# jackyko1991/vnet-tensorflow

Hardware: AMD Instinct MI355X
Metric: training patches/sec (128^3x1ch fp32) (higher is better)
Workload: dtype f32

## Files before the change

### vnet_tensorflow_amd/_lib.py

```python
import ctypes
import os
import subprocess

_HERE = os.path.dirname(os.path.abspath(__file__))
LIB_PATH = os.environ.get("VNET_HIP_LIB") or os.path.join(_HERE, "libvnet_hip.so")
CSRC = os.path.join(_HERE, "csrc")

_vp, _i, _i64, _f, _sz, _u64, _d = (ctypes.c_void_p, ctypes.c_int, ctypes.c_int64, ctypes.c_float,
                                    ctypes.c_size_t, ctypes.c_uint64, ctypes.c_double)

SIGNATURES = {
    "vnet_version": (ctypes.c_char_p, []),
    "vnet_set_option": (_d, [ctypes.c_char_p, _d]),
    "vnet_get_option": (_d, [ctypes.c_char_p]),
    "vnet_packed_weight_floats": (_sz, [_i, _i, _i, _i]),
    "vnet_pack_weights": (_i, [_i, _vp, _vp, _i, _i, _i, _vp]),
    "vnet_packed_dims": (_i, [_i, _i, _i, _i, ctypes.POINTER(ctypes.c_int), ctypes.POINTER(ctypes.c_int)]),
    "vnet_pack_weights_batched": (_i, [_vp, _i, _vp]),
    "vnet_conv_x3_ok": (_i, [_i] * 8),
    "vnet_conv_x3_stats_rows": (_i, [_i] * 6),
    "vnet_conv_x3_ws_bytes": (_sz, [_i] * 6),
    "vnet_conv_fwd_x3": (_i, [_vp, _i, _vp, _i, _vp, _vp, _vp, _i, _vp, _i, _i, _i, _i, _i, _vp, _vp, _vp, _vp, _sz, _vp]),
    "vnet_wgrad_x3_ok": (_i, [_i] * 7),
    "vnet_wgrad_x3_ws_bytes": (_sz, [_i] * 6),
# ... 85 lines not shown
    "vnet_bn_act_bwd_apply_b16": (_i, [_vp, _vp, _vp, _i, _i64, _i, _vp, _vp, _vp, _vp, _i, _vp, _vp, _vp, _d, _vp, _vp, _vp]),
    "vnet_bn_small_ok": (_i, [_i64, _i]),
    "vnet_bn_small_fwd_b16": (_i, [_vp, _vp, _i64, _i, _f, _f, _vp, _vp, _i, _vp, _vp, _vp, _vp, _vp, _vp, _vp]),
    "vnet_bn_small_bwd_b16": (_i, [_vp, _vp, _vp, _i64, _i, _vp, _vp, _vp, _vp, _i, _vp, _vp, _vp, _vp, _vp, _vp]),
    "vnet_head_fwd_b16": (_i, [_vp, _vp, _vp, _vp, _i64, _i, _i, _vp]),
    "vnet_head_bwd_b16": (_i, [_vp, _vp, _vp, _vp, _vp, _vp, _i64, _i, _i, _vp, _sz, _vp]),
    "vnet_dropout_fwd_b16": (_i, [_vp, _vp, _vp, _i64, _f, _u64, _vp, _vp]),
    "vnet_dropout_bwd_b16": (_i, [_vp, _vp, _vp, _i64, _f, _vp]),
}

SIGNATURES_UNET = {
    "vnet_maxpool2_fwd": (_i, [_vp, _vp, _i, _i, _i, _i, _i, _vp]),
    "vnet_maxpool2_bwd": (_i, [_vp, _vp, _vp, _vp, _i, _i, _i, _i, _i, _i, _vp]),
}


class WgradJob(ctypes.Structure):
    _fields_ = [("x0", ctypes.c_void_p), ("x1", ctypes.c_void_p), ("dy", ctypes.c_void_p), ("dw", ctypes.c_void_p),
                ("ws", ctypes.c_void_p), ("ws_bytes", ctypes.c_size_t),
                ("C0", ctypes.c_int), ("C1", ctypes.c_int), ("Cout", ctypes.c_int), ("Cin_dw", ctypes.c_int),
                ("B", ctypes.c_int), ("D", ctypes.c_int), ("H", ctypes.c_int), ("W", ctypes.c_int), ("ks", ctypes.c_int)]


ERRORS = {-1: "VNET_E_BADARG", -2: "VNET_E_UNSUPPORTED", -3: "VNET_E_WORKSPACE"}


def set_option(name, value):
    prev = lib().vnet_set_option(name.encode(), float(value))
    if prev != prev:
        raise VnetHipError("unknown library option %r" % (name,))
# ... 21 lines not shown
def lib():
    global _lib
    if _lib is None:
        if not os.path.exists(LIB_PATH):
            raise VnetHipError("libvnet_hip.so not found at %s -- run `python -c 'import __graft_entry__ as g; g.build()'` "
                               "(hipcc, gfx950).  The HIP library is the only compute path." % LIB_PATH)
        import torch
        L = ctypes.CDLL(LIB_PATH)
        for name, (res, args) in SIGNATURES.items():
            fn = getattr(L, name)
            fn.restype, fn.argtypes = res, args
            if name == "vnet_conv_b16_stats_rows":
                setattr(L, name, _memo(fn, (b"BF16_DEEP", b"BF16_DEEP_TARGET"), L))
            elif name.endswith("_ws_bytes") or name.endswith("_stats_rows") or name == "vnet_conv_stats_from_reduce" or name == "vnet_packed_weight_floats":
                setattr(L, name, _memo(fn))
        for name, (res, args) in SIGNATURES_UNET.items():
            fn = getattr(L, name)
            fn.restype, fn.argtypes = res, args
        _lib = L
    return _lib


_MEMOS = []


def _memo(fn, opts=None, L=None):
    cache = {}
    _MEMOS.append(cache)

    def cached(*args):
        key = args if opts is None else args + tuple(L.vnet_get_option(o) for o in opts)
        r = cache.get(key)
        if r is None:
# ... 9 lines not shown
```

### vnet_tensorflow_amd/csrc/elementwise.hip

```cpp
#include "common.h"

namespace {

#ifndef VNET_BN_RED_U
#define VNET_BN_RED_U 2
#endif
constexpr int EW_BLOCK = 256;
#ifndef VNET_EW_MAXBLK
#define VNET_EW_MAXBLK 1024
#endif
constexpr int EW_MAXBLK = VNET_EW_MAXBLK;
constexpr int MAXC = 1024;

inline int ew_blocks(size_t work_items) {
    size_t b = (work_items + EW_BLOCK - 1) / EW_BLOCK;
    if (b < 1) b = 1;
    if (b > EW_MAXBLK) b = EW_MAXBLK;
    return (int)b;
}
inline bool is_pow2(int v) { return v > 0 && (v & (v - 1)) == 0; }

__device__ __forceinline__ float act_fwd(float z, int act, float al) {
    if (act == VNET_ACT_RELU) return fmaxf(z, 0.f);
    if (act == VNET_ACT_PRELU) return fmaxf(z, 0.f) + al * fminf(z, 0.f);
// ... 485 lines not shown
        const float4 v = x[idx];
        acc[0].x += v.x; acc[0].y += v.y; acc[0].z += v.z; acc[0].w += v.w;
    }
    block_reduce_vec<1>(acc, CQ, CQ * 4, partial + (size_t)blockIdx.x * CQ * 4);
}
__global__ void __launch_bounds__(EW_BLOCK) colsum_generic_kernel(const float* __restrict__ x, size_t n, int C, float* __restrict__ partial) {
    __shared__ float sh[MAXC];
    for (int c = threadIdx.x; c < C; c += EW_BLOCK) sh[c] = 0.f;
    __syncthreads();
    const size_t stride = (size_t)gridDim.x * EW_BLOCK;
    for (size_t idx = (size_t)blockIdx.x * EW_BLOCK + threadIdx.x; idx < n; idx += stride) atomicAdd(&sh[idx % C], x[idx]);
    __syncthreads();
    for (int c = threadIdx.x; c < C; c += EW_BLOCK) partial[(size_t)blockIdx.x * C + c] = sh[c];
}

template <int K>
__global__ void __launch_bounds__(EW_BLOCK) head_fwd_kernel(const float* __restrict__ x, const float* __restrict__ w,
                                                            const float* __restrict__ bias, float* __restrict__ y, size_t M, int C) {
    __shared__ float ws[MAXC * 8 / 8];
    for (int t = threadIdx.x; t < C * K; t += EW_BLOCK) ws[t] = w[t];
    __syncthreads();
    const size_t stride = (size_t)gridDim.x * EW_BLOCK;
    for (size_t row = (size_t)blockIdx.x * EW_BLOCK + threadIdx.x; row < M; row += stride) {
        float o[K];
#pragma unroll
        for (int k = 0; k < K; ++k) o[k] = bias ? bias[k] : 0.f;
        const float* xr = x + row * C;
        if ((C & 3) == 0) {
            for (int c = 0; c < C; c += 4) {
                const float4 v = *reinterpret_cast<const float4*>(xr + c);
#pragma unroll
                for (int k = 0; k < K; ++k)
                    o[k] += v.x * ws[c * K + k] + v.y * ws[(c + 1) * K + k] + v.z * ws[(c + 2) * K + k] + v.w * ws[(c + 3) * K + k];
            }
        } else {
            for (int c = 0; c < C; ++c) {
                const float v = xr[c];
#pragma unroll
                for (int k = 0; k < K; ++k) o[k] += v * ws[c * K + k];
            }
        }
#pragma unroll
        for (int k = 0; k < K; ++k) y[row * K + k] = o[k];
    }
}

template <int K>
__global__ void __launch_bounds__(EW_BLOCK) head_bwd_kernel(const float* __restrict__ x, const float* __restrict__ w,
// ... 55 lines not shown
    for (size_t row = (size_t)blockIdx.x * EW_BLOCK + threadIdx.x; row < M; row += stride) {
        float g[K];
#pragma unroll
        for (int k = 0; k < K; ++k) { g[k] = dy[row * K + k]; atomicAdd(&acc[C * K + k], g[k]); }
        for (int c = 0; c < C; ++c) {
            const float v = x[row * C + c];
            float o = 0.f;
#pragma unroll
            for (int k = 0; k < K; ++k) { o += g[k] * ws[c * K + k]; atomicAdd(&acc[c * K + k], v * g[k]); }
            if (dx) dx[row * C + c] = o;
        }
    }
    __syncthreads();
    float* prow = partial + (size_t)blockIdx.x * (C * K + K);
    for (int t = threadIdx.x; t < C * K + K; t += EW_BLOCK) prow[t] = acc[t];
}

struct LossP {
    const float* logits; const int32_t* labels; const float* weights;
    float* softmax_out; long long* pred_out; float* partial;
    size_t V; int B; int K; int kind; int nblk;
};

template <int K>
__global__ void __launch_bounds__(EW_BLOCK) softmax_dice_fwd_kernel(LossP p) {
    const int b = blockIdx.y;
    const bool jac = (p.kind & 15) == VNET_LOSS_JACCARD;
    const bool wx = (p.kind & VNET_LOSS_WEIGHTED) && p.weights;
    float aI[K], aL[K], aR[K], aX = 0.f;
#pragma unroll
// ... 893 lines not shown
    const float sc = 1.f / (1.f - rate);
    for (size_t i = (size_t)blockIdx.x * blockDim.x + threadIdx.x; i < n8; i += (size_t)gridDim.x * blockDim.x) {
        float v[8];
        unpack8(dy[i], v);
        const uint2 m = reinterpret_cast<const uint2*>(mask)[i];
#pragma unroll
        for (int k = 0; k < 8; ++k) v[k] = (((k < 4 ? m.x : m.y) >> (8 * (k & 3))) & 0xffu) ? v[k] * sc : 0.f;
        dx[i] = pack8(v);
    }
}
}

template <typename F>
static int with_k(int K, F&& f) { return with_int<1, 2, 3, 4, 5, 6, 7, 8>(K, f); }
template <typename F>
static int with_bcast_r(bool bcast, bool hasr, F&& f) {
    return bcast ? f(std::true_type{}, std::false_type{}) : with_bool(hasr, [&](auto R) { return f(std::false_type{}, R); });
}

extern "C" {

size_t vnet_bn_ws_bytes(int C) { return (size_t)EW_MAXBLK * 3 * (C > 8 ? C : 8) * sizeof(float); }
size_t vnet_colsum_ws_bytes(int C) { return (size_t)EW_MAXBLK * (C > 8 ? C : 8) * sizeof(float); }
size_t vnet_head_ws_bytes(int C, int K) { return (size_t)EW_MAXBLK * (C * K + K) * sizeof(float); }
size_t vnet_loss_ws_bytes(int B, int K) { return (size_t)B * EW_MAXBLK * (3 * K + 1) * sizeof(float) + (size_t)B * (3 * K + 1) * sizeof(double) + 16; }

static int bn_partial_moments(const float* x, const float* r, int bcast, int64_t M, int C, float* partial, hipStream_t st, int* nblk_out) {
    const int Cs = bcast ? 1 : C;
    const int mode = red_mode(Cs);
    int nblk, e;
// ... 215 lines not shown
    float* partial = (float*)ws;
    int nblk, e;
    if ((C & 3) == 0 && is_pow2(C / 4) && C / 4 <= EW_BLOCK) {
        nblk = ew_blocks((size_t)M * (C / 4) / 4 + 1);
        e = with_k(K, [&](auto KK) {
            return launch<head_bwd_kernel<KK>>(dim3(nblk), dim3(EW_BLOCK), 0, st, x, w, dy, dx, (size_t)M, C, partial);
        });
    } else {
        nblk = ew_blocks((size_t)M / 4 + 1);
        e = with_k(K, [&](auto KK) {
            return launch<head_bwd_generic_kernel<KK>>(dim3(nblk), dim3(EW_BLOCK), 0, st, x, w, dy, dx, (size_t)M, C, partial);
        });
    }
    if (e) return e;
    return launch<head_finalize_kernel>(dim3(C * K + K), dim3(256), 0, st, partial, nblk, C * K, K, dw, db);
}

int vnet_softmax_dice_fwd(const float* logits, const int32_t* labels, int B, int64_t V, int K,
                          int loss_kind, const float* weights, float alpha, float smooth,
                          float* softmax_out, int64_t* pred_out, float* loss_out, float* dice_out,
                          float* coef, void* ws, size_t ws_bytes, void* stream) {
    if (!logits || !labels || !loss_out || !coef || B <= 0 || V <= 0 || K <= 0) return VNET_E_BADARG;
    if (B * K > 64 || B > 8) return VNET_E_UNSUPPORTED;
    if ((loss_kind & 15) > VNET_LOSS_XENT) return VNET_E_UNSUPPORTED;
    if ((loss_kind & VNET_LOSS_WEIGHTED) && !weights) return VNET_E_BADARG;
    if (!ws || ws_bytes < vnet_loss_ws_bytes(B, K)) return VNET_E_WORKSPACE;
    hipStream_t st = (hipStream_t)stream;
    LossP p{}; p.logits = logits; p.labels = labels; p.weights = weights; p.softmax_out = softmax_out;
    p.pred_out = (long long*)pred_out; p.partial = (float*)ws; p.V = (size_t)V; p.B = B; p.K = K; p.kind = loss_kind;
    const int nblk = ew_blocks((size_t)V / 4 + 1);
// ... 331 lines not shown
```

### vnet_tensorflow_amd/layers2.py

```python
import numpy as np

from . import ops
from ._scope import get_variable, variable_scope, current


def xavier_initializer_convolution(shape, dist='uniform', lambda_initializer=True):
    s = len(shape) - 2
    num_activations = np.prod(shape[:s]) * np.sum(shape[s:])
    if dist == 'uniform':
        lim = np.sqrt(6. / num_activations)
        return np.random.uniform(-lim, lim, shape).astype(np.float32)
    if dist == 'normal':
        stddev = np.sqrt(3. / num_activations)
        return np.random.normal(0, stddev, shape).astype(np.float32)
    raise ValueError('Distribution must be either "uniform" or "normal".')


def constant_initializer(value, shape, lambda_initializer=True):
    return np.full(shape, value).astype(np.float32)


def get_num_channels(x):
    return int(x.shape[-1])

# ... 101 lines not shown
    return ops.activation(x, "relu")


def leaky_relu(x):
    return ops.activation(x, "lrelu")


def convolution_tiled(tiled, filter, bn_stats=False, bn_residual=None):
    filter = list(filter)
    w = get_variable(name='weights', initializer=lambda: xavier_initializer_convolution(shape=filter))
    b = get_variable(name='biases', initializer=lambda: constant_initializer(0, shape=filter[-1]))
    img, gamma, beta, mean, invstd = tiled
    return ops.input_conv(img, gamma, beta, mean, invstd, w, b, bn_stats=bn_stats, bn_residual=bn_residual)


def batch_normalization(x, activation=None, residual=None, tile=False, channels=None, dead=False,
                        momentum=0.99, epsilon=0.001, want_stats=False):
    C = int(channels if channels is not None else x.shape[-1])
    gamma, beta, mm, mv = _bn_variables(C)
    if dead:
        ops.bn_update_only(x, C, mm, mv)
        return None
    alpha = None
    if activation == "prelu":
        alpha = get_variable('alpha', initializer=lambda: np.full((C,), 0.1, dtype=np.float32))
    if want_stats:
        y, mean, invstd = ops.bn_act(x, gamma, beta, activation, alpha, residual, tile, mm, mv, want_stats=True)
        return y, (x, gamma, beta, mean, invstd)
    return ops.bn_act(x, gamma, beta, activation, alpha, residual, tile, mm, mv)


def _bn_variables(C):
    store = current()
    with variable_scope(store.unique_layer_name("batch_normalization")):
        gamma = get_variable('gamma', initializer=lambda: np.ones((C,), np.float32))
        beta = get_variable('beta', initializer=lambda: np.zeros((C,), np.float32))
        mm = get_variable('moving_mean', initializer=lambda: np.zeros((C,), np.float32), trainable=False)
        mv = get_variable('moving_variance', initializer=lambda: np.ones((C,), np.float32), trainable=False)
    return gamma, beta, mm, mv


def batch_normalization_chain(x, kind, activation=None):
    C = int(x.shape[-1])
    layers = [_bn_variables(C) for _ in range(3 if kind == 0 else 2)]
    alpha = None
    if activation == "prelu":
        alpha = get_variable('alpha', initializer=lambda: np.full((C,), 0.1, dtype=np.float32))
    (g1, b1, mm1, mv1), (g2, b2, mm2, mv2) = layers[0], layers[1]
    g3 = b3 = mm3 = mv3 = None
    if kind == 0:
        g3, b3, mm3, mv3 = layers[2]
    return ops.bn_chain(x, kind, activation, alpha, g1, b1, g2, b2, g3, b3, (mm1, mv1, mm2, mv2, mm3, mv3))
```

### vnet_tensorflow_amd/networks.py

```python
import torch

from . import layers2 as L
from ._scope import VariableStore


class VNet(object):
    def __init__(self,
                 num_classes,
                 dropout_rate=0.01,
                 num_channels=16,
                 num_levels=4,
                 num_convolutions=(1, 2, 3, 3),
                 bottom_convolutions=3,
                 is_training=True,
                 activation_fn="relu",
                 device=None):
        self.num_classes = num_classes
        self.dropout_rate = dropout_rate
        self.num_channels = num_channels
        assert num_levels == len(num_convolutions)
        self.num_levels = num_levels
        self.num_convolutions = num_convolutions
        self.bottom_convolutions = bottom_convolutions
        self.is_training = is_training
        self.train_phase = True
        if activation_fn not in ("relu", "prelu", "lrelu"):
            raise ValueError("activation_fn must be relu, prelu or lrelu")
        self.activation_fn = activation_fn
        self.fuse_input_block = True
        self.fuse_bn_chains = True
        self.cut_backward = False
        self.backward_cuts = []
        self.fuse_bn_stats = True
        self.fuse_grad_accumulation = True
        self.fuse_zero_bias_grad = True
        self.variables = VariableStore(device)

    def parameters(self):
        return list(self.variables.params.values())

    def named_parameters(self):
        return list(self.variables.params.items())

    def state_dict(self):
        return self.variables.state_dict()

    def load_state_dict(self, sd):
        self.variables.load_state_dict(sd)

    def build(self, input_shape):
# ... 49 lines not shown
                        x = L.down_convolution(x, factor=2, kernel_size=[2, 2, 2], bn_stats=self.fuse_bn_stats)
                        x = L.batch_normalization(x, activation=act)

            if cutting:
                features = [ops.cut(f, self.backward_cuts) for f in features]
                x = ops.cut(x, self.backward_cuts)
            with store.variable_scope('vnet/bottom_level'):
                x = self.convolution_block(x, self.bottom_convolutions, dropout_rate, act)

            for l in reversed(range(self.num_levels)):
                with store.variable_scope('vnet/decoder/level_' + str(l + 1)):
                    f = features[l]
                    with store.variable_scope('up_convolution'):
                        x = L.up_convolution(x, tuple(f.shape), factor=2, kernel_size=[2, 2, 2])
                        x = L.batch_normalization(x, activation=act)
                    x = self.convolution_block_2(x, f, self.num_convolutions[l], dropout_rate, act)

            with store.variable_scope('vnet/output_layer'):
                logits = L.convolution(x, [1, 1, 1, self.num_channels, self.num_classes])
                logits = L.batch_normalization(logits)
        return logits

    def convolution_block(self, layer_input, num_convolutions, dropout_rate, activation_fn, is_training=True, tiled=None):
        from . import ops
        store = self.variables
        x = layer_input
        n_channels = L.get_num_channels(x)
        if tiled is None and self.fuse_grad_accumulation:
            x, layer_input = ops.fork(layer_input)
        for i in range(num_convolutions):
            with store.variable_scope('conv_' + str(i + 1)):
                res = layer_input if i == num_convolutions - 1 else None
                if i == 0 and tiled is not None:
                    x = L.convolution_tiled(tiled, [5, 5, 5, n_channels, n_channels], bn_stats=self.fuse_bn_stats, bn_residual=res)
                else:
                    x = L.convolution(x, [5, 5, 5, n_channels, n_channels], bn_stats=self.fuse_bn_stats, bn_residual=res)
                x = L.batch_normalization(x, activation=activation_fn, residual=res)
                x = ops.dropout(x, dropout_rate)
        return x

    def convolution_block_2(self, layer_input, fine_grained_features, num_convolutions, dropout_rate, activation_fn,
                            is_training=True):
        from . import ops
        store = self.variables
        n_channels = L.get_num_channels(layer_input)
        if num_convolutions == 1:
            with store.variable_scope('conv_' + str(1)):
                x = L.convolution_concat(layer_input, fine_grained_features, [5, 5, 5, n_channels * 2, n_channels], bn_stats=self.fuse_bn_stats)
                if self.fuse_bn_chains:
                    x = L.batch_normalization_chain(x, 0, activation_fn)
                else:
                    x = L.batch_normalization(x)
                    r = L.batch_normalization(x)
                    x = L.batch_normalization(x, activation=activation_fn, residual=r)
                x = ops.dropout(x, dropout_rate)
            return x

        with store.variable_scope('conv_' + str(1)):
            x = L.convolution_concat(layer_input, fine_grained_features, [5, 5, 5, n_channels * 2, n_channels], bn_stats=self.fuse_bn_stats)
            x = L.batch_normalization(x, activation=activation_fn)
            x = ops.dropout(x, dropout_rate)

        for i in range(1, num_convolutions):
            with store.variable_scope('conv_' + str(i + 1)):
                x = L.convolution(x, [5, 5, 5, n_channels, n_channels], bn_stats=self.fuse_bn_stats)
                last = (i == num_convolutions - 1)
                if last and self.fuse_bn_chains:
                    x = L.batch_normalization_chain(x, 1, activation_fn)
                else:
                    r = L.batch_normalization(x, dead=not last)
                    x = L.batch_normalization(x, activation=activation_fn, residual=r if last else None)
                x = ops.dropout(x, dropout_rate)
        return x


class UNet(object):

    def __init__(self,
                 num_output_channels,
                 dropout_rate=0.01,
                 num_channels=4,
                 num_levels=4,
                 num_convolutions=2,
                 bottom_convolutions=2,
                 is_training=True,
                 activation_fn="relu",
                 device=None):
# ... 102 lines not shown
```

### vnet_tensorflow_amd/ops.py

```python
import collections
import contextlib
import ctypes
import math
import os as _os
import weakref

import torch

from . import _lib
from ._lib import VnetHipError, check

BN_EPS = 1e-3
BN_MOMENTUM = 0.99

ACT = {None: 0, "none": 0, "relu": 1, "prelu": 2, "lrelu": 3}
PACK_FWD, PACK_BWD, PACK_UP, PACK_FWD_BF16, PACK_BWD_BF16, PACK_BOTH_BF16, PACK_BOTH = 0, 1, 2, 3, 4, 5, 6
PACK_FWD_X3, PACK_BWD_X3, PACK_BOTH_X3 = 7, 8, 9

class OpsContext(object):
    def __init__(self):
        self.compute = {"dtype": "fp32", "store16": False, "name": "fp32", "split3": False}
        self.pg = {"on": False, "streams": {}, "used": set(), "keep": []}
        self.pack_epoch = [0]
        self.pack_reg = {"entries": [], "descs": None, "device": None}
# ... 1022 lines not shown
        name = "vnet_bn_stats" + sfx
        check(getattr(L, name)(_ptr(x), _ptr(r), *tile, M, C, BN_EPS, BN_MOMENTUM, _ptr(mean), _ptr(invstd), _ptr(mm), _ptr(mv),
                               _ptr(ws), nb, _stream()), name)
        return mean, invstd, float(M)
    all_reduce, world = _SYNC_BN
    sums = torch.empty(2 * C, dtype=torch.float64, device=x.device)
    name = "vnet_bn_moments" + sfx
    check(getattr(L, name)(_ptr(x), _ptr(r), *tile, M, C, _ptr(sums), _ptr(ws), nb, _stream()), name)
    all_reduce(sums)
    check(L.vnet_bn_finalize(_ptr(sums), float(M) * world, C, BN_EPS, BN_MOMENTUM, _ptr(mean), _ptr(invstd),
                             _ptr(mm), _ptr(mv), _stream()), "vnet_bn_finalize")
    return mean, invstd, float(M) * world


def _bn_backward(rt, dy, x, r, bcast, M, C, mean, invstd, scale, shift, act, alpha, dscale, dshift, dalpha, ds, m_total,
                 all_reduce=None, coef=None):
    L = _lib.lib()
    nb = L.vnet_bn_ws_bytes(C)
    ws = workspace(nb, dy.device)
    if rt.stats == "small":
        check(L.vnet_bn_small_bwd_b16(_ptr(dy), _ptr(x), _ptr(r), M, C, _ptr(mean), _ptr(invstd), _ptr(scale), _ptr(shift), act,
                                      _ptr(alpha), _ptr(dscale), _ptr(dshift), _ptr(dalpha), _ptr(ds), _stream()), "vnet_bn_small_bwd_b16")
        return
    sfx = "_b16" if rt.apply16 else ""
    args = (_ptr(dy), _ptr(x), _ptr(r), int(bcast), M, C, _ptr(mean), _ptr(invstd), _ptr(scale), _ptr(shift), act, _ptr(alpha))
    name = "vnet_bn_act_bwd_reduce" + sfx
    check(getattr(L, name)(*args, _ptr(dscale), _ptr(dshift), _ptr(dalpha), _ptr(ws), nb, _stream()), name)
    sdz, sdzx = dshift, dscale
    if rt.allreduce and (ds is not None or coef is not None):
        sdz = torch.cat([dshift.reshape(-1), dscale.reshape(-1)])
        all_reduce(sdz)
        sdzx = sdz[C:]
    extra = coef(sdzx) if coef is not None else None
    if ds is not None:
        name = "vnet_bn_act_bwd_apply" + sfx
        check(getattr(L, name)(*args, _ptr(sdz), _ptr(sdzx), m_total, _ptr(extra), _ptr(ds), _stream()), name)


class _BnActFn(torch.autograd.Function):
    @staticmethod
    def forward(ctx, x, r, gamma, beta, alpha, act, bcast, mm, mv):
        L = _lib.lib()
# ... 311 lines not shown
            check(L.vnet_head_bwd_b16(_ptr(x), _ptr(w), _ptr(dy), _ptr(dx), _ptr(dw), _ptr(db), M, C, K, _ptr(ws), nb, _stream()),
                  "vnet_head_bwd_b16")
        else:
            check(L.vnet_head_bwd(_ptr(x), _ptr(w), _ptr(dy), _ptr(dx), _ptr(dw), _ptr(db), M, C, K, _ptr(ws), nb, _stream()),
                  "vnet_head_bwd")
        return dx, _grad_ret(dw, sw), _grad_ret(db, sb)


def head_conv(x, w, b):
    if _meta(x):
        return torch.empty(x.shape[:-1] + (w.shape[-1],), device="meta")
    _need_gpu(x, "head_conv", allow16=True)
    return _HeadFn.apply(x, w, b)


def parse_loss(name):
    valid = ("xent", "weighted_xent", "sorensen", "weighted_sorensen", "jaccard", "weighted_jaccard",
             "mixed_sorensen", "mixed_weighted_sorensen", "mixed_jaccard", "mixed_weighted_jaccard")
    if name not in valid:
        raise SystemExit("Invalid loss function")
    kind = LOSS_KIND["xent"] if name.endswith("xent") else (LOSS_KIND["sorensen"] if "sorensen" in name else LOSS_KIND["jaccard"])
    if "weighted" in name:
        kind |= LOSS_WEIGHTED
    if name.startswith("mixed_"):
        kind |= LOSS_MIXED
    return kind


_CONST_VEC = {}

# ... 240 lines not shown
```

Measured before the change: 65.46.

## Fuse final batch-norm+activation with the 1x1 head convolution in forward and backward

Adds fused HIP kernels that apply batch-norm plus activation and immediately compute the 1x1x1 head logits, so the normalized activation tensor is never written out for small channel counts (C=8 or 16). The backward path is fused too: one reduce kernel computes the BN gradient sums together with the head weight and bias gradients, and one apply kernel recomputes dy from dlogits and the head weights on the fly. The goal is to remove full-volume reads and writes of the intermediate activation and its gradient, plus several kernel launches. In exchange the kernels use cross-lane shuffles and larger per-thread register footprints, and the forward head dot product disables FMA contraction to match the unfused numerics.

```diff
diff --git a/include/vnet_hip_head.h b/include/vnet_hip_head.h
--- /dev/null
+++ b/include/vnet_hip_head.h
@@ -0,0 +1,28 @@
+#ifndef VNET_HIP_HEAD_H
+#define VNET_HIP_HEAD_H
+#include "vnet_hip.h"
+
+#ifdef __cplusplus
+extern "C" {
+#endif
+
+int vnet_bn_head_ok(int C, int K);
+int vnet_bn_head_stats_rows(int64_t M, int C);
+size_t vnet_bn_head_ws_bytes(int C, int K);
+
+int vnet_bn_act_head_fwd(const float* x, const float* r, int64_t M, int C,
+    const float* mean, const float* invstd, const float* gamma, const float* beta, int act, const float* alpha,
+    const float* w, const float* bias, int K, float* y, float* logits, float* stats, void* stream);
+
+int vnet_bn_act_bwd_reduce_head(const float* dlogits, const float* w, int K, const float* x, const float* r, int64_t M, int C,
+    const float* mean, const float* invstd, const float* gamma, const float* beta, int act, const float* alpha,
+    float* dgamma, float* dbeta, float* dalpha, float* dw, float* db, void* ws, size_t ws_bytes, void* stream);
+
+int vnet_bn_act_bwd_apply_head(const float* dlogits, const float* w, int K, const float* x, const float* r, int64_t M, int C,
+    const float* mean, const float* invstd, const float* gamma, const float* beta, int act, const float* alpha,
+    const float* sum_dz, const float* sum_dz_xhat, double M_total, const float* xhat_coef, float* ds, void* stream);
+
+#ifdef __cplusplus
+}
+#endif
+#endif
diff --git a/vnet_tensorflow_amd/_lib.py b/vnet_tensorflow_amd/_lib.py
--- a/vnet_tensorflow_amd/_lib.py
+++ b/vnet_tensorflow_amd/_lib.py
@@ -123,6 +123,16 @@
     "vnet_maxpool2_bwd": (_i, [_vp, _vp, _vp, _vp, _i, _i, _i, _i, _i, _i, _vp]),
 }
 
+SIGNATURES_HEAD = {
+    "vnet_bn_head_ok": (_i, [_i, _i]),
+    "vnet_bn_head_stats_rows": (_i, [_i64, _i]),
+    "vnet_bn_head_ws_bytes": (_sz, [_i, _i]),
+    "vnet_bn_act_head_fwd": (_i, [_vp, _vp, _i64, _i, _vp, _vp, _vp, _vp, _i, _vp, _vp, _vp, _i, _vp, _vp, _vp, _vp]),
+    "vnet_bn_act_bwd_reduce_head": (_i, [_vp, _vp, _i, _vp, _vp, _i64, _i, _vp, _vp, _vp, _vp, _i, _vp,
+                                         _vp, _vp, _vp, _vp, _vp, _vp, _sz, _vp]),
+    "vnet_bn_act_bwd_apply_head": (_i, [_vp, _vp, _i, _vp, _vp, _i64, _i, _vp, _vp, _vp, _vp, _i, _vp, _vp, _vp, _d, _vp, _vp, _vp]),
+}
+
 
 class WgradJob(ctypes.Structure):
     _fields_ = [("x0", ctypes.c_void_p), ("x1", ctypes.c_void_p), ("dy", ctypes.c_void_p), ("dw", ctypes.c_void_p),
@@ -174,9 +184,11 @@
                 setattr(L, name, _memo(fn, (b"BF16_DEEP", b"BF16_DEEP_TARGET"), L))
             elif name.endswith("_ws_bytes") or name.endswith("_stats_rows") or name == "vnet_conv_stats_from_reduce" or name == "vnet_packed_weight_floats":
                 setattr(L, name, _memo(fn))
-        for name, (res, args) in SIGNATURES_UNET.items():
+        for name, (res, args) in list(SIGNATURES_UNET.items()) + list(SIGNATURES_HEAD.items()):
             fn = getattr(L, name)
             fn.restype, fn.argtypes = res, args
+            if name in ("vnet_bn_head_ok", "vnet_bn_head_stats_rows", "vnet_bn_head_ws_bytes"):
+                setattr(L, name, _memo(fn))
         _lib = L
     return _lib
 
diff --git a/vnet_tensorflow_amd/csrc/elementwise.hip b/vnet_tensorflow_amd/csrc/elementwise.hip
--- a/vnet_tensorflow_amd/csrc/elementwise.hip
+++ b/vnet_tensorflow_amd/csrc/elementwise.hip
@@ -1,4 +1,5 @@
 #include "common.h"
+#include "../../include/vnet_hip_head.h"
 
 namespace {
 
@@ -523,6 +524,10 @@
     for (int c = threadIdx.x; c < C; c += EW_BLOCK) partial[(size_t)blockIdx.x * C + c] = sh[c];
 }
 
+__device__ __forceinline__ float head_quad_dot(const float4 v, float w0, float w1, float w2, float w3) {
+#pragma clang fp contract(off)
+    return v.x * w0 + v.y * w1 + v.z * w2 + v.w * w3;
+}
 template <int K>
 __global__ void __launch_bounds__(EW_BLOCK) head_fwd_kernel(const float* __restrict__ x, const float* __restrict__ w,
                                                             const float* __restrict__ bias, float* __restrict__ y, size_t M, int C) {
@@ -539,8 +544,7 @@
             for (int c = 0; c < C; c += 4) {
                 const float4 v = *reinterpret_cast<const float4*>(xr + c);
 #pragma unroll
-                for (int k = 0; k < K; ++k)
-                    o[k] += v.x * ws[c * K + k] + v.y * ws[(c + 1) * K + k] + v.z * ws[(c + 2) * K + k] + v.w * ws[(c + 3) * K + k];
+                for (int k = 0; k < K; ++k) o[k] += head_quad_dot(v, ws[c * K + k], ws[(c + 1) * K + k], ws[(c + 2) * K + k], ws[(c + 3) * K + k]);
             }
         } else {
             for (int c = 0; c < C; ++c) {
@@ -626,6 +630,218 @@
     __syncthreads();
     float* prow = partial + (size_t)blockIdx.x * (C * K + K);
     for (int t = threadIdx.x; t < C * K + K; t += EW_BLOCK) prow[t] = acc[t];
+}
+
+struct HeadP {
+    const float* w; const float* bias; const float* dl;
+    float* logits; float* stats; float* hpartial;
+};
+
+template <int K>
+__device__ __forceinline__ void head_load_row(const float* __restrict__ p, size_t row, float (&g)[K]) {
+    if constexpr (K == 2) { const float2 t = reinterpret_cast<const float2*>(p)[row]; g[0] = t.x; g[1] = t.y; }
+    else if constexpr (K == 4) { const float4 t = reinterpret_cast<const float4*>(p)[row]; g[0] = t.x; g[1] = t.y; g[2] = t.z; g[3] = t.w; }
+    else {
+#pragma unroll
+        for (int k = 0; k < K; ++k) g[k] = p[row * K + k];
+    }
+}
+template <int K>
+__device__ __forceinline__ void head_store_row(float* __restrict__ p, size_t row, const float (&g)[K]) {
+    if constexpr (K == 2) reinterpret_cast<float2*>(p)[row] = make_float2(g[0], g[1]);
+    else if constexpr (K == 4) reinterpret_cast<float4*>(p)[row] = make_float4(g[0], g[1], g[2], g[3]);
+    else {
+#pragma unroll
+        for (int k = 0; k < K; ++k) p[row * K + k] = g[k];
+    }
+}
+
+struct HeadQuad { float sc[4], sf[4], al[4], mu[4], is[4]; };
+template <int K>
+__device__ __forceinline__ void head_quad_load(const BnP& p, const HeadP& h, int c, const float* sc, const float* sf, const float* al,
+                                               HeadQuad& q, float (&wv)[4][K]) {
+#pragma unroll
+    for (int i = 0; i < 4; ++i) {
+        q.sc[i] = sc[c + i]; q.sf[i] = sf[c + i]; q.al[i] = al[c + i];
+        q.mu[i] = p.mean[c + i]; q.is[i] = p.invstd[c + i];
+#pragma unroll
+        for (int k = 0; k < K; ++k) wv[i][k] = h.w[(c + i) * K + k];
+    }
+}
+template <int K>
+__device__ __forceinline__ void head_quad_dy(const float (&g)[K], const float (&wv)[4][K], float (&dy)[4]) {
+    float4 o = make_float4(0, 0, 0, 0);
+#pragma unroll
+    for (int k = 0; k < K; ++k) {
+        o.x = fmaf(g[k], wv[0][k], o.x); o.y = fmaf(g[k], wv[1][k], o.y);
+        o.z = fmaf(g[k], wv[2][k], o.z); o.w = fmaf(g[k], wv[3][k], o.w);
+    }
+    dy[0] = o.x; dy[1] = o.y; dy[2] = o.z; dy[3] = o.w;
+}
+
+template <int K, int CQ>
+__global__ void __launch_bounds__(EW_BLOCK) bn_act_head_fwd_kernel(BnP p, HeadP h) {
+    __shared__ float sc[MAXC], sf[MAXC], al[MAXC];
+    bn_load_coef(p, sc, sf, al);
+    const size_t nq = p.M * CQ;
+    const size_t stride = (size_t)gridDim.x * EW_BLOCK;
+    const size_t start = (size_t)blockIdx.x * EW_BLOCK + threadIdx.x;
+    const int cq = (int)(start % CQ), c = cq * 4;
+    HeadQuad q; float wv[4][K], bias[K];
+    head_quad_load<K>(p, h, c, sc, sf, al, q, wv);
+#pragma unroll
+    for (int k = 0; k < K; ++k) bias[k] = h.bias ? h.bias[k] : 0.f;
+    float acc[2][8];
+#pragma unroll
+    for (int k = 0; k < 8; ++k) acc[0][k] = acc[1][k] = 0.f;
+    for (size_t idx = start; idx < nq; idx += stride) {
+        float4 v = reinterpret_cast<const float4*>(p.x)[idx];
+        if (p.r) { const float4 t = reinterpret_cast<const float4*>(p.r)[idx]; v.x += t.x; v.y += t.y; v.z += t.z; v.w += t.w; }
+        float4 o;
+        o.x = act_fwd(v.x * q.sc[0] + q.sf[0], p.act, q.al[0]);
+        o.y = act_fwd(v.y * q.sc[1] + q.sf[1], p.act, q.al[1]);
+        o.z = act_fwd(v.z * q.sc[2] + q.sf[2], p.act, q.al[2]);
+        o.w = act_fwd(v.w * q.sc[3] + q.sf[3], p.act, q.al[3]);
+        if (p.out) reinterpret_cast<float4*>(p.out)[idx] = o;
+        float part[K], lg[K];
+#pragma unroll
+        for (int k = 0; k < K; ++k) { part[k] = head_quad_dot(o, wv[0][k], wv[1][k], wv[2][k], wv[3][k]); lg[k] = bias[k]; }
+#pragma unroll
+        for (int j = 0; j < CQ; ++j)
+#pragma unroll
+            for (int k = 0; k < K; ++k) lg[k] += __shfl(part[k], j, CQ);
+        if (cq == 0) {
+            head_store_row<K>(h.logits, idx / CQ, lg);
+#pragma unroll
+            for (int k = 0; k < K; ++k) { acc[0][k] += lg[k]; acc[1][k] += lg[k] * lg[k]; }
+        }
+    }
+    if (h.stats) block_reduce_row<2, 8>(acc, K, h.stats + (size_t)blockIdx.x * 2 * K);
+}
+
+template <int K, int CQ>
+__global__ void __launch_bounds__(EW_BLOCK) bn_act_bwd_reduce_head_kernel(BnP p, HeadP h) {
+    __shared__ float sc[MAXC], sf[MAXC], al[MAXC];
+    __shared__ float shh[5 * K][EW_BLOCK];
+    bn_load_coef(p, sc, sf, al);
+    constexpr int C = 4 * CQ;
+    const size_t nq = p.M * CQ;
+    const size_t stride = (size_t)gridDim.x * EW_BLOCK;
+    const size_t start = (size_t)blockIdx.x * EW_BLOCK + threadIdx.x;
+    const int cq = (int)(start % CQ), c = cq * 4;
+    HeadQuad q; float wv[4][K];
+    head_quad_load<K>(p, h, c, sc, sf, al, q, wv);
+    float4 acc[3] = {make_float4(0, 0, 0, 0), make_float4(0, 0, 0, 0), make_float4(0, 0, 0, 0)};
+    float hs[5 * K];
+#pragma unroll
+    for (int s = 0; s < 5 * K; ++s) hs[s] = 0.f;
+    constexpr int U = VNET_BN_RED_U;
+    for (size_t idx = start; idx < nq; idx += U * stride) {
+        float4 v[U]; float g[U][K];
+#pragma unroll
+        for (int u = 0; u < U; ++u) {
+            const size_t j0 = idx + u * stride;
+            const bool ok = j0 < nq;
+            const size_t j = ok ? j0 : idx;
+            v[u] = reinterpret_cast<const float4*>(p.x)[j];
+            if (p.r) { const float4 t = reinterpret_cast<const float4*>(p.r)[j]; v[u].x += t.x; v[u].y += t.y; v[u].z += t.z; v[u].w += t.w; }
+            head_load_row<K>(h.dl, j / CQ, g[u]);
+            if (!ok) {
+#pragma unroll
+                for (int k = 0; k < K; ++k) g[u][k] = 0.f;
+            }
+        }
+#pragma unroll
+        for (int u = 0; u < U; ++u) {
+            const float vv[4] = {v[u].x, v[u].y, v[u].z, v[u].w};
+            float gg[4], a0[4], a1[4], a2[4];
+            head_quad_dy<K>(g[u], wv, gg);
+#pragma unroll
+            for (int i = 0; i < 4; ++i) {
+                const float z = vv[i] * q.sc[i] + q.sf[i];
+                const float dz = gg[i] * act_grad(z, p.act, q.al[i]);
+                const float xh = (vv[i] - q.mu[i]) * q.is[i];
+                a0[i] = dz; a1[i] = dz * xh; a2[i] = gg[i] * fminf(z, 0.f);
+                const float y = act_fwd(z, p.act, q.al[i]);
+#pragma unroll
+                for (int k = 0; k < K; ++k) hs[i * K + k] = fmaf(y, g[u][k], hs[i * K + k]);
+            }
+            acc[0].x += a0[0]; acc[0].y += a0[1]; acc[0].z += a0[2]; acc[0].w += a0[3];
+            acc[1].x += a1[0]; acc[1].y += a1[1]; acc[1].z += a1[2]; acc[1].w += a1[3];
+            acc[2].x += a2[0]; acc[2].y += a2[1]; acc[2].z += a2[2]; acc[2].w += a2[3];
+            if (cq == 0) {
+#pragma unroll
+                for (int k = 0; k < K; ++k) hs[4 * K + k] += g[u][k];
+            }
+        }
+    }
+    block_reduce_vec<3>(acc, CQ, C, p.partial + (size_t)blockIdx.x * 3 * C);
+#pragma unroll
+    for (int s = 0; s < 5 * K; ++s) shh[s][threadIdx.x] = hs[s];
+    __syncthreads();
+    if (threadIdx.x < 64) {
+        const int t = threadIdx.x;
+        float* prow = h.hpartial + (size_t)blockIdx.x * (C * K + K);
+#pragma unroll
+        for (int s = 0; s < 5 * K; ++s) {
+            float v = (shh[s][t] + shh[s][t + 128]) + (shh[s][t + 64] + shh[s][t + 192]);
+#pragma unroll
+            for (int o = 32; o >= CQ; o >>= 1) v += __shfl_down(v, o, 64);
+            if (s < 4 * K) { if (t < CQ) prow[(t * 4 + s / K) * K + s % K] = v; }
+            else if (t == 0) prow[C * K + s - 4 * K] = v;
+        }
+    }
+}
+
+template <int K, int CQ>
+__global__ void __launch_bounds__(EW_BLOCK) bn_act_bwd_apply_head_kernel(BnP p, HeadP h) {
+    __shared__ float sc[MAXC], sf[MAXC], al[MAXC];
+    bn_load_coef(p, sc, sf, al);
+    const size_t nq = p.M * CQ;
+    const size_t stride = (size_t)gridDim.x * EW_BLOCK;
+    const size_t start = (size_t)blockIdx.x * EW_BLOCK + threadIdx.x;
+    const int cq = (int)(start % CQ), c = cq * 4;
+    HeadQuad q; float wv[4][K], k1[4], k2[4], ex[4];
+    head_quad_load<K>(p, h, c, sc, sf, al, q, wv);
+#pragma unroll
+    for (int i = 0; i < 4; ++i) {
+        k1[i] = p.dbeta[c + i] * p.invM; k2[i] = p.dgamma[c + i] * p.invM;
+        ex[i] = p.extra ? p.extra[c + i] : 0.f;
+    }
+    for (size_t idx = start; idx < nq; idx += stride) {
+        float4 v = reinterpret_cast<const float4*>(p.x)[idx];
+        if (p.r) { const float4 t = reinterpret_cast<const float4*>(p.r)[idx]; v.x += t.x; v.y += t.y; v.z += t.z; v.w += t.w; }
+        float g[K], gg[4], o[4];
+        head_load_row<K>(h.dl, idx / CQ, g);
+        head_quad_dy<K>(g, wv, gg);
+        const float vv[4] = {v.x, v.y, v.z, v.w};
+#pragma unroll
+        for (int i = 0; i < 4; ++i) {
+            const float z = vv[i] * q.sc[i] + q.sf[i];
+            const float dz = gg[i] * act_grad(z, p.act, q.al[i]);
+            const float xh = (vv[i] - q.mu[i]) * q.is[i];
+            o[i] = q.sc[i] * (dz - k1[i] - xh * k2[i]) + xh * ex[i];
+        }
+        reinterpret_cast<float4*>(p.out)[idx] = make_float4(o[0], o[1], o[2], o[3]);
+    }
+}
+
+__global__ void __launch_bounds__(256) bn_head_finalize_kernel(const float* __restrict__ bnp, const float* __restrict__ hp, int nblk,
+                                                               int C, int CK, int K, float* o0, float* o1, float* o2, float* dw, float* db) {
+    if ((int)blockIdx.x < C) {
+        const int c = blockIdx.x;
+        double s[3];
+        block_colsum_multi<3>(bnp, nblk, (size_t)3 * C, c, C, s);
+        if (threadIdx.x == 0) {
+            if (o0) o0[c] = (float)s[0];
+            if (o1) o1[c] = (float)s[1];
+            if (o2) o2[c] = (float)s[2];
+        }
+        return;
+    }
+    const int c = blockIdx.x - C;
+    const double s = block_colsum_d(hp, nblk, (size_t)(CK + K), c);
+    if (threadIdx.x == 0) { if (c < CK) dw[c] = (float)s; else db[c - CK] = (float)s; }
 }
 
 struct LossP {
@@ -1549,6 +1765,10 @@
 template <typename F>
 static int with_k(int K, F&& f) { return with_int<1, 2, 3, 4, 5, 6, 7, 8>(K, f); }
 template <typename F>
+static int with_k_cq(int K, int C, F&& f) {
+    return with_k(K, [&](auto KK) { return with_int<2, 4>(C / 4, [&](auto CQ) { return f(KK, CQ); }); });
+}
+template <typename F>
 static int with_bcast_r(bool bcast, bool hasr, F&& f) {
     return bcast ? f(std::true_type{}, std::false_type{}) : with_bool(hasr, [&](auto R) { return f(std::false_type{}, R); });
 }
@@ -1794,6 +2014,65 @@
     }
     if (e) return e;
     return launch<head_finalize_kernel>(dim3(C * K + K), dim3(256), 0, st, partial, nblk, C * K, K, dw, db);
+}
+
+static inline bool bn_head_shape_ok(int C, int K) { return (C == 8 || C == 16) && K >= 1 && K <= 8; }
+static inline int bn_head_blocks(int64_t M, int C) { return ew_blocks((size_t)M * C / 4 / 4 + 1); }
+
+int vnet_bn_head_ok(int C, int K) { return bn_head_shape_ok(C, K) ? 1 : 0; }
+int vnet_bn_head_stats_rows(int64_t M, int C) { return (M > 0 && (C == 8 || C == 16)) ? bn_head_blocks(M, C) : 0; }
+size_t vnet_bn_head_ws_bytes(int C, int K) { return (size_t)EW_MAXBLK * (3 * C + C * K + K) * sizeof(float); }
+
+int vnet_bn_act_head_fwd(const float* x, const float* r, int64_t M, int C,
+                         const float* mean, const float* invstd, const float* gamma, const float* beta, int act, const float* alpha,
+                         const float* w, const float* bias, int K, float* y, float* logits, float* stats, void* stream) {
+    if (!x || !mean || !invstd || !gamma || !beta || !w || !logits || M <= 0) return VNET_E_BADARG;
+    if (act == VNET_ACT_PRELU && !alpha) return VNET_E_BADARG;
+    if (act < 0 || act > 3 || !bn_head_shape_ok(C, K)) return VNET_E_UNSUPPORTED;
+    BnP p{}; p.x = x; p.r = r; p.mean = mean; p.invstd = invstd; p.gamma = gamma; p.beta = beta; p.alpha = alpha;
+    p.out = y; p.M = (size_t)M; p.C = C; p.act = act;
+    HeadP h{}; h.w = w; h.bias = bias; h.logits = logits; h.stats = stats;
+    return with_k_cq(K, C, [&](auto KK, auto CQ) {
+        return launch<bn_act_head_fwd_kernel<KK, CQ>>(dim3(bn_head_blocks(M, C)), dim3(EW_BLOCK), 0, (hipStream_t)stream, p, h);
+    });
+}
+
+int vnet_bn_act_bwd_reduce_head(const float* dlogits, const float* w, int K, const float* x, const float* r, int64_t M, int C,
+                                const float* mean, const float* invstd, const float* gamma, const float* beta,
+                                int act, const float* alpha, float* dgamma, float* dbeta, float* dalpha, float* dw, float* db,
+                                void* ws, size_t ws_bytes, void* stream) {
+    if (!dlogits || !w || !x || !mean || !invstd || !gamma || !beta || !dgamma || !dbeta || !dw || !db || M <= 0) return VNET_E_BADARG;
+    if (act == VNET_ACT_PRELU && (!alpha || !dalpha)) return VNET_E_BADARG;
+    if (act < 0 || act > 3 || !bn_head_shape_ok(C, K)) return VNET_E_UNSUPPORTED;
+    if (!ws || ws_bytes < vnet_bn_head_ws_bytes(C, K)) return VNET_E_WORKSPACE;
+    hipStream_t st = (hipStream_t)stream;
+    BnP p{}; bn_bwd_fill(p, nullptr, x, r, 0, M, C, mean, invstd, gamma, beta, act, alpha);
+    p.partial = (float*)ws;
+    HeadP h{}; h.w = w; h.dl = dlogits; h.hpartial = p.partial + (size_t)EW_MAXBLK * 3 * C;
+    const int nblk = bn_head_blocks(M, C);
+    if (int e = with_k_cq(K, C, [&](auto KK, auto CQ) {
+            return launch<bn_act_bwd_reduce_head_kernel<KK, CQ>>(dim3(nblk), dim3(EW_BLOCK), 0, st, p, h); }))
+        return e;
+    return launch<bn_head_finalize_kernel>(dim3(C + C * K + K), dim3(256), 0, st, (const float*)p.partial, (const float*)h.hpartial, nblk,
+                                           C, C * K, K, dbeta, dgamma, act == VNET_ACT_PRELU ? dalpha : (float*)nullptr, dw, db);
+}
+
+int vnet_bn_act_bwd_apply_head(const float* dlogits, const float* w, int K, const float* x, const float* r, int64_t M, int C,
+                               const float* mean, const float* invstd, const float* gamma, const float* beta,
+                               int act, const float* alpha, const float* sum_dz, const float* sum_dz_xhat, double M_total,
+                               const float* xhat_coef, float* ds, void* stream) {
+    if (!dlogits || !w || !x || !mean || !invstd || !gamma || !beta || !sum_dz || !sum_dz_xhat || !ds || M <= 0 || M_total <= 0.0)
+        return VNET_E_BADARG;
+    if (act == VNET_ACT_PRELU && !alpha) return VNET_E_BADARG;
+    if (act < 0 || act > 3 || !bn_head_shape_ok(C, K)) return VNET_E_UNSUPPORTED;
+    BnP p{}; bn_bwd_fill(p, nullptr, x, r, 0, M, C, mean, invstd, gamma, beta, act, alpha);
+    p.invM = (float)(1.0 / M_total);
+    p.extra = xhat_coef;
+    p.out = ds; p.dgamma = sum_dz_xhat; p.dbeta = sum_dz;
+    HeadP h{}; h.w = w; h.dl = dlogits;
+    return with_k_cq(K, C, [&](auto KK, auto CQ) {
+        return launch<bn_act_bwd_apply_head_kernel<KK, CQ>>(dim3(bn_head_blocks(M, C)), dim3(EW_BLOCK), 0, (hipStream_t)stream, p, h);
+    });
 }
 
 int vnet_softmax_dice_fwd(const float* logits, const int32_t* labels, int B, int64_t V, int K,
diff --git a/vnet_tensorflow_amd/layers2.py b/vnet_tensorflow_amd/layers2.py
--- a/vnet_tensorflow_amd/layers2.py
+++ b/vnet_tensorflow_amd/layers2.py
@@ -139,8 +139,25 @@
     return ops.input_conv(img, gamma, beta, mean, invstd, w, b, bn_stats=bn_stats, bn_residual=bn_residual)
 
 
+class DeferredNorm(object):
+
+    def __init__(self, x, kind, activation, alpha, layers, residual=None):
+        self.x, self.kind, self.activation, self.alpha, self.layers, self.residual = x, kind, activation, alpha, layers, residual
+        self.shape = x.shape
+
+
+def convolution_after_norm(d, filter):
+    filter = list(filter)
+    assert filter[:3] == [1, 1, 1], filter
+    w = get_variable(name='weights', initializer=lambda: xavier_initializer_convolution(shape=filter))
+    b = get_variable(name='biases', initializer=lambda: constant_initializer(0, shape=filter[-1]))
+    g = [v for layer in d.layers for v in layer[:2]] + [None] * (6 - 2 * len(d.layers))
+    moving = [v for layer in d.layers for v in layer[2:]] + [None] * (6 - 2 * len(d.layers))
+    return ops.bn_head(d.x, w, b, d.kind, d.activation, d.alpha, *g, residual=d.residual, moving=tuple(moving))
+
+
 def batch_normalization(x, activation=None, residual=None, tile=False, channels=None, dead=False,
-                        momentum=0.99, epsilon=0.001, want_stats=False):
+                        momentum=0.99, epsilon=0.001, want_stats=False, defer=False):
     C = int(channels if channels is not None else x.shape[-1])
     gamma, beta, mm, mv = _bn_variables(C)
     if dead:
@@ -149,6 +166,9 @@
     alpha = None
     if activation == "prelu":
         alpha = get_variable('alpha', initializer=lambda: np.full((C,), 0.1, dtype=np.float32))
+    if defer:
+        assert not tile and not want_stats
+        return DeferredNorm(x, -1, activation, alpha, [(gamma, beta, mm, mv)], residual)
     if want_stats:
         y, mean, invstd = ops.bn_act(x, gamma, beta, activation, alpha, residual, tile, mm, mv, want_stats=True)
         return y, (x, gamma, beta, mean, invstd)
@@ -165,12 +185,14 @@
     return gamma, beta, mm, mv
 
 
-def batch_normalization_chain(x, kind, activation=None):
+def batch_normalization_chain(x, kind, activation=None, defer=False):
     C = int(x.shape[-1])
     layers = [_bn_variables(C) for _ in range(3 if kind == 0 else 2)]
     alpha = None
     if activation == "prelu":
         alpha = get_variable('alpha', initializer=lambda: np.full((C,), 0.1, dtype=np.float32))
+    if defer:
+        return DeferredNorm(x, kind, activation, alpha, layers)
     (g1, b1, mm1, mv1), (g2, b2, mm2, mv2) = layers[0], layers[1]
     g3 = b3 = mm3 = mv3 = None
     if kind == 0:
diff --git a/vnet_tensorflow_amd/networks.py b/vnet_tensorflow_amd/networks.py
--- a/vnet_tensorflow_amd/networks.py
+++ b/vnet_tensorflow_amd/networks.py
@@ -34,6 +34,7 @@
         self.fuse_bn_stats = True
         self.fuse_grad_accumulation = True
         self.fuse_zero_bias_grad = True
+        self.fuse_head = True
         self.variables = VariableStore(device)
 
     def parameters(self):
@@ -113,10 +114,14 @@
                     with store.variable_scope('up_convolution'):
                         x = L.up_convolution(x, tuple(f.shape), factor=2, kernel_size=[2, 2, 2])
                         x = L.batch_normalization(x, activation=act)
-                    x = self.convolution_block_2(x, f, self.num_convolutions[l], dropout_rate, act)
+                    x = self.convolution_block_2(x, f, self.num_convolutions[l], dropout_rate, act,
+                                                 head=(l == 0 and self.fuse_head))
 
             with store.variable_scope('vnet/output_layer'):
-                logits = L.convolution(x, [1, 1, 1, self.num_channels, self.num_classes])
+                if isinstance(x, L.DeferredNorm):
+                    logits = L.convolution_after_norm(x, [1, 1, 1, self.num_channels, self.num_classes])
+                else:
+                    logits = L.convolution(x, [1, 1, 1, self.num_channels, self.num_classes])
                 logits = L.batch_normalization(logits)
         return logits
 
@@ -139,20 +144,22 @@
         return x
 
     def convolution_block_2(self, layer_input, fine_grained_features, num_convolutions, dropout_rate, activation_fn,
-                            is_training=True):
+                            is_training=True, head=False):
         from . import ops
         store = self.variables
         n_channels = L.get_num_channels(layer_input)
+        defer = bool(head) and dropout_rate == 0.0
         if num_convolutions == 1:
             with store.variable_scope('conv_' + str(1)):
                 x = L.convolution_concat(layer_input, fine_grained_features, [5, 5, 5, n_channels * 2, n_channels], bn_stats=self.fuse_bn_stats)
                 if self.fuse_bn_chains:
-                    x = L.batch_normalization_chain(x, 0, activation_fn)
+                    x = L.batch_normalization_chain(x, 0, activation_fn, defer=defer)
                 else:
                     x = L.batch_normalization(x)
                     r = L.batch_normalization(x)
-                    x = L.batch_normalization(x, activation=activation_fn, residual=r)
-                x = ops.dropout(x, dropout_rate)
+                    x = L.batch_normalization(x, activation=activation_fn, residual=r, defer=defer)
+                if not defer:
+                    x = ops.dropout(x, dropout_rate)
             return x
 
         with store.variable_scope('conv_' + str(1)):
@@ -165,11 +172,12 @@
                 x = L.convolution(x, [5, 5, 5, n_channels, n_channels], bn_stats=self.fuse_bn_stats)
                 last = (i == num_convolutions - 1)
                 if last and self.fuse_bn_chains:
-                    x = L.batch_normalization_chain(x, 1, activation_fn)
+                    x = L.batch_normalization_chain(x, 1, activation_fn, defer=defer)
                 else:
                     r = L.batch_normalization(x, dead=not last)
-                    x = L.batch_normalization(x, activation=activation_fn, residual=r if last else None)
-                x = ops.dropout(x, dropout_rate)
+                    x = L.batch_normalization(x, activation=activation_fn, residual=r if last else None, defer=defer and last)
+                if not (defer and last):
+                    x = ops.dropout(x, dropout_rate)
         return x
 
 
diff --git a/vnet_tensorflow_amd/ops.py b/vnet_tensorflow_amd/ops.py
--- a/vnet_tensorflow_amd/ops.py
+++ b/vnet_tensorflow_amd/ops.py
@@ -1060,18 +1060,28 @@
 
 
 def _bn_backward(rt, dy, x, r, bcast, M, C, mean, invstd, scale, shift, act, alpha, dscale, dshift, dalpha, ds, m_total,
-                 all_reduce=None, coef=None):
+                 all_reduce=None, coef=None, head=None):
     L = _lib.lib()
-    nb = L.vnet_bn_ws_bytes(C)
-    ws = workspace(nb, dy.device)
-    if rt.stats == "small":
-        check(L.vnet_bn_small_bwd_b16(_ptr(dy), _ptr(x), _ptr(r), M, C, _ptr(mean), _ptr(invstd), _ptr(scale), _ptr(shift), act,
-                                      _ptr(alpha), _ptr(dscale), _ptr(dshift), _ptr(dalpha), _ptr(ds), _stream()), "vnet_bn_small_bwd_b16")
-        return
-    sfx = "_b16" if rt.apply16 else ""
-    args = (_ptr(dy), _ptr(x), _ptr(r), int(bcast), M, C, _ptr(mean), _ptr(invstd), _ptr(scale), _ptr(shift), act, _ptr(alpha))
-    name = "vnet_bn_act_bwd_reduce" + sfx
-    check(getattr(L, name)(*args, _ptr(dscale), _ptr(dshift), _ptr(dalpha), _ptr(ws), nb, _stream()), name)
+    if head is not None:
+        w, dw, db = head
+        K = int(w.shape[-1])
+        nb = L.vnet_bn_head_ws_bytes(C, K)
+        ws = workspace(nb, dy.device)
+        sfx = "_head"
+        args = (_ptr(dy), _ptr(w), K, _ptr(x), _ptr(r), M, C, _ptr(mean), _ptr(invstd), _ptr(scale), _ptr(shift), act, _ptr(alpha))
+        check(L.vnet_bn_act_bwd_reduce_head(*args, _ptr(dscale), _ptr(dshift), _ptr(dalpha), _ptr(dw), _ptr(db), _ptr(ws), nb, _stream()),
+              "vnet_bn_act_bwd_reduce_head")
+    else:
+        nb = L.vnet_bn_ws_bytes(C)
+        ws = workspace(nb, dy.device)
+        if rt.stats == "small":
+            check(L.vnet_bn_small_bwd_b16(_ptr(dy), _ptr(x), _ptr(r), M, C, _ptr(mean), _ptr(invstd), _ptr(scale), _ptr(shift), act,
+                                          _ptr(alpha), _ptr(dscale), _ptr(dshift), _ptr(dalpha), _ptr(ds), _stream()), "vnet_bn_small_bwd_b16")
+            return
+        sfx = "_b16" if rt.apply16 else ""
+        args = (_ptr(dy), _ptr(x), _ptr(r), int(bcast), M, C, _ptr(mean), _ptr(invstd), _ptr(scale), _ptr(shift), act, _ptr(alpha))
+        name = "vnet_bn_act_bwd_reduce" + sfx
+        check(getattr(L, name)(*args, _ptr(dscale), _ptr(dshift), _ptr(dalpha), _ptr(ws), nb, _stream()), name)
     sdz, sdzx = dshift, dscale
     if rt.allreduce and (ds is not None or coef is not None):
         sdz = torch.cat([dshift.reshape(-1), dscale.reshape(-1)])
@@ -1413,6 +1423,115 @@
     return _HeadFn.apply(x, w, b)
 
 
+_HEAD_FUSE = {"on": True, "stats": False}
+
+
+def set_head_fusion(on, stats=None):
+    prev = (_HEAD_FUSE["on"], _HEAD_FUSE["stats"])
+    _HEAD_FUSE["on"] = bool(on)
+    if stats is not None:
+        _HEAD_FUSE["stats"] = bool(stats)
+    return prev
+
+
+class _BnHeadFn(torch.autograd.Function):
+
+    @staticmethod
+    def forward(ctx, x, r, kind, act, alpha, w, b, stats, bufs, g1, b1, g2, b2, g3, b3):
+        L = _lib.lib()
+        C, K = int(w.shape[-2]), int(w.shape[-1])
+        pre = _epilogue_of(x, r, C)
+        x = x.contiguous()
+        r = r.contiguous() if r is not None else None
+        M = x.numel() // C
+        dev = x.device
+        mm1, mv1, mm2, mv2, mm3, mv3 = bufs
+        if kind < 0:
+            ctx.rt = rt = bn_route("act", M, C, False, False, None if r is None else False, pre is not None)
+        else:
+            ctx.rt = rt = bn_route("chain", M, C, x16=False, epilogue=pre is not None)
+        mean, invstd, ctx.m_total = _bn_stats(rt, x, r, False, M, C, mm1, mv1, pre)
+        ctx.all_reduce = _SYNC_BN[0] if rt.allreduce else None
+        scale, shift = g1, b1
+        if kind >= 0:
+            scale = torch.empty(C, dtype=torch.float32, device=dev)
+            shift = torch.empty(C, dtype=torch.float32, device=dev)
+            check(L.vnet_bn_chain_coef_fwd(kind, C, BN_EPS, BN_MOMENTUM, _ptr(mean), _ptr(invstd), _ptr(g1), _ptr(b1), _ptr(g2), _ptr(b2),
+                                           _ptr(g3), _ptr(b3), _ptr(scale), _ptr(shift), _ptr(mm2), _ptr(mv2), _ptr(mm3), _ptr(mv3),
+                                           _stream()), "vnet_bn_chain_coef_fwd")
+        logits = torch.empty(x.shape[:-1] + (K,), dtype=torch.float32, device=dev)
+        check(L.vnet_bn_act_head_fwd(_ptr(x), _ptr(r), M, C, _ptr(mean), _ptr(invstd), _ptr(scale), _ptr(shift), act, _ptr(alpha),
+                                     _ptr(w), _ptr(b), K, None, _ptr(logits), _ptr(stats), _stream()), "vnet_bn_act_head_fwd")
+        ctx.save_for_backward(x, r, alpha, w, g1, g2, g3, mean, invstd, scale, shift)
+        ctx.params = (alpha, w, b, g1, b1, g2, b2, g3, b3)
+        ctx.cfg = (kind, act, M, C)
+        return logits
+
+    @staticmethod
+    def backward(ctx, dl):
+        L = _lib.lib()
+        x, r, alpha, w, g1, g2, g3, mean, invstd, scale, shift = ctx.saved_tensors
+        kind, act, M, C = ctx.cfg
+        aref, wref, bref, g1r, b1r, g2r, b2r, g3r, b3r = ctx.params
+        dl = dl.contiguous()
+        dev = dl.device
+        dw, sw = _grad_out(wref)
+        db, sb = _grad_out(bref)
+        dalpha, sa = _grad_out(aref) if alpha is not None else (None, None)
+        need_ds = ctx.needs_input_grad[0] or (r is not None and ctx.needs_input_grad[1])
+        ds = torch.empty(x.shape, dtype=torch.float32, device=dev) if need_ds else None
+        outs = [_grad_out(p) if p is not None else (None, None) for p in (g1r, b1r, g2r, b2r, g3r, b3r)]
+        (dg1, s1), (db1, t1), (dg2, s2), (db2, t2), (dg3, s3), (db3, t3) = outs
+        if kind < 0:
+            _bn_backward(ctx.rt, dl, x, r, False, M, C, mean, invstd, scale, shift, act, alpha, dg1, db1, dalpha, ds, ctx.m_total,
+                         ctx.all_reduce, head=(w, dw, db))
+        else:
+            dC = torch.empty(C, dtype=torch.float32, device=dev)
+            dD = torch.empty(C, dtype=torch.float32, device=dev)
+            extra = torch.empty(C, dtype=torch.float32, device=dev)
+
+            def coef(dCg):
+                check(L.vnet_bn_chain_coef_bwd(kind, C, BN_EPS, ctx.m_total, _ptr(mean), _ptr(invstd), _ptr(g1), _ptr(g2), _ptr(g3),
+                                               _ptr(dC), _ptr(dD), _ptr(dCg), _ptr(dg1), _ptr(db1), _ptr(dg2), _ptr(db2), _ptr(dg3),
+                                               _ptr(db3), _ptr(extra), _stream()), "vnet_bn_chain_coef_bwd")
+                return extra
+            _bn_backward(ctx.rt, dl, x, None, False, M, C, mean, invstd, scale, shift, act, alpha, dC, dD, dalpha, ds, ctx.m_total,
+                         ctx.all_reduce, coef, head=(w, dw, db))
+        ret = [_grad_ret(g, s_) if p is not None else None
+               for g, s_, p in ((dg1, s1, g1r), (db1, t1, b1r), (dg2, s2, g2r), (db2, t2, b2r), (dg3, s3, g3r), (db3, t3, b3r))]
+        return (ds, (ds if r is not None else None), None, None, _grad_ret(dalpha, sa) if alpha is not None else None,
+                _grad_ret(dw, sw), _grad_ret(db, sb), None, None) + tuple(ret)
+
+
+def bn_head(x, w, b, kind, act, alpha, g1, b1, g2=None, b2=None, g3=None, b3=None, residual=None, moving=(None,) * 6):
+    a = ACT[act]
+    K = int(w.shape[-1])
+    C = int(w.shape[-2])
+    if _meta(x):
+        return torch.empty(x.shape[:-1] + (K,), device="meta")
+    fused = (_HEAD_FUSE["on"] and x.dtype == torch.float32 and not storage_is_bf16() and (residual is None or residual.dtype == torch.float32)
+             and int(x.shape[-1]) == C and (kind < 0 or residual is None) and _lib.lib().vnet_bn_head_ok(C, K))
+    if not fused:
+        if kind < 0:
+            y = bn_act(x, g1, b1, act, alpha, residual, False, moving[0], moving[1])
+        else:
+            y = bn_chain(x, kind, act, alpha, g1, b1, g2, b2, g3, b3, moving)
+        return head_conv(y, w, b)
+    _need_gpu(x, "bn_head")
+    if a == 2 and alpha is None:
+        raise VnetHipError("prelu needs alpha")
+    if kind == 0 and (g3 is None or b3 is None):
+        raise VnetHipError("bn_chain kind 0 needs three batch-norm layers")
+    stats = rows = None
+    if _HEAD_FUSE["stats"] and _SYNC_BN is None:
+        rows = _lib.lib().vnet_bn_head_stats_rows(x.numel() // C, C)
+        stats = torch.empty((rows, 2 * K), dtype=torch.float32, device=x.device)
+    logits = _BnHeadFn.apply(x, residual, int(kind), a, alpha if a == 2 else None, w, b, stats, tuple(moving), g1, b1, g2, b2, g3, b3)
+    if stats is not None:
+        logits._vnet_stats = _EpilogueStats(stats, rows, None)
+    return logits
+
+
 def parse_loss(name):
     valid = ("xent", "weighted_xent", "sorensen", "weighted_sorensen", "jaccard", "weighted_jaccard",
              "mixed_sorensen", "mixed_weighted_sorensen", "mixed_jaccard", "mixed_weighted_jaccard")
```

New measurement: 66.62, median of 6. 1.8% higher.
